# yulong314/multi_camera_calibration

Hardware: AMD Instinct MI355X
Metric: corner residual+Jacobian evals/sec + ms/LM-iter; RMS reproj-err vs ref (higher is better)
Workload: dtype f64; 1 GPU; config4: 4 omnidirectional cameras, 1000 synthetic 11x8-board views (BASELINE.json configs[3]), one Gauss-Newton step per 'step'; model=omnidirectional, cameras=4, views=1000, edges=3958, params=6018, parallelism=photo-sharded x1, transport=none, state_dtype=f32, jacobian_dtype=f64

## Files before the change

### multi_camera_calibration_amd/csrc/mcc_group.hpp

```cpp


template <int MODEL, bool BACK, int L, int GW = 28>
__device__ __forceinline__ void group_prologue(const double* ph, const double* ct, const double* sds, int side,
                                               int sub, double* S, double* P, double* Gb) {
    const double* R1 = ph;
    const double* Jr1 = ph + 9;
    const double* T1 = ph + 18;
    const double* R2 = ct;
    const double* Jl2 = ct + 9;
    const double* T2 = ct + 18;
    double* X = S;
    double* W = S + 15;
    for (int e = sub; e < 12; e += L) {
        if (e < 9) {
            const int i = e / 3, j = e % 3;
            X[e] = dot3_nc(R2[i * 3], R1[j], R2[i * 3 + 1], R1[3 + j], R2[i * 3 + 2], R1[6 + j]);
        } else {
            const int i = e - 9;
            const double q = dot3_nc(R2[i * 3], T1[0], R2[i * 3 + 1], T1[1], R2[i * 3 + 2], T1[2]);
            X[12 + i] = q;
            X[9 + i] = add_nc(q, T2[i]);
        }
    }
    wave_sync_lds();
// ... 351 lines not shown
    const int iter = st->iter;
    const double cn0 = st->cam_normG2, cn1 = st->cam_normX2;
    const int nI = 48 * np, nV = useiv ? m * m + 1 : 0, n = nI + nV;
    if (tid == 0) {
        s_status = useiv ? 0.0 : -1.0;
        s_fail = 0;
    }
    __syncthreads();
    unsigned have = 0;
    auto due = [&](int t) { return t >= nI || t < 48 * a.n_items || t % 48 < 3; };
    const long long t0 = (long long)__builtin_amdgcn_s_memrealtime();
    for (;;) {
        double v[U];
#pragma unroll
        for (int u = 0; u < U; ++u) {
            int t = u * nt + tid;
            t = t < n ? t : n - 1;
            v[u] = ld_sc1(t < nI ? a.item_out + t : la.fiv + (t - nI));
        }
        const double stt = useiv ? ld_sc1(la.fiv + m * m) : -1.0;
        int pend = 0;
#pragma unroll
        for (int u = 0; u < U; ++u) {
            const int t = u * nt + tid;
            if (t >= n || ((have >> u) & 1) || !due(t)) continue;
            if (!fold_valid(v[u])) {
                if (t < nI || t == nI + m * m || !fold_valid(stt) || stt > 0.0) ++pend;
                continue;
            }
            have |= 1u << u;
            if (t < nI) itm[t] = v[u];
            else if (t < nI + m * m) Iv[t - nI] = v[u];
            else s_status = v[u];
        }
        if (!__syncthreads_or(pend)) break;
        if (tid == 0 && (long long)__builtin_amdgcn_s_memrealtime() - t0 >= la.spare_wait) {
            atomicOr(&st->error, kErrWarmTimeout);
            st->done = 1;
            s_fail = 1;
        }
        __syncthreads();
        if (s_fail) return;
    }
#pragma unroll
    for (int u = 0; u < U; ++u) {
        const int t = u * nt + tid;
        if (t < n && ((have >> u) & 1)) fold_empty(t < nI ? a.item_out + t : la.fiv + (t - nI));
    }
    if (tid <= a.nblk) sbi[tid] = bi;
    int err_now = 0;
    for (int k = a.n_items; k < np; ++k) err_now |= itm[48 * k + 2] != 0.0 ? kErrPhotoNotPD : 0;
    __syncthreads();
    SSTAMP(srow, 8, 0);
    schur_finish(a, np, iter, cn0, cn1, err_now, useiv && s_status == (double)(iter + 1), srow, pre);
}
constexpr int kFoldKI = 8;
__device__ __forceinline__ void fold_final_reset(const LinArgs& la, const double* const* src, unsigned have, bool useiv) {
#pragma unroll
    for (int q = 0; q < kFoldKI; ++q)
        if ((have >> q) & 1) fold_empty(const_cast<double*>(src[q]));
    if (threadIdx.x == 0 && useiv) fold_empty(la.fiv + la.fsa.m * la.fsa.m);
}
__device__ __forceinline__ void fold_final_direct(const LinArgs& la, const SolvePre* pre) {
    const SchurArgs& a = la.fsa;
    State* st = a.state;
    const int tid = threadIdx.x, nt = blockDim.x;
    const int m = a.m, nb = m / 6, ntri = m * (m + 1) / 2, np = la.fold_parts, nc = np - a.n_items;
    extern __shared__ __attribute__((aligned(16))) double sm[];
    double* S = sm;
    double* r = sm + m * m;
    double* Iv = sm + m * m + m;
    __shared__ double norms[2];
    __shared__ int s_fail;
    const bool useiv = a.ssinv != nullptr && a.fuse_solve;
    const bool lds = a.fuse_solve && a.peer.nranks == 0;
    long long* srow = a.stamps ? a.stamps + kSchurStampStride * (size_t)np : nullptr;
    SSTAMP(srow, 10, 0);
    const int nent = a.nblk * 48, ivt0 = nent + 2, nivt = nt - ivt0;
    const double* src[kFoldKI];
    int cnt = 0, kind = 0;
    int blk = 0, e = 0;
    if (tid < nent) {
        blk = tid / 48;
        e = tid % 48;
        const int k0 = a.block_items[blk], nk = a.block_items[blk + 1] - k0;
        int b1 = 0;
#pragma unroll
        for (int b = 1; b < 5; ++b)
            if (b < nb && b * nb - b * (b - 1) / 2 <= blk) b1 = b;
        const int b2 = b1 + (blk - (b1 * nb - b1 * (b1 - 1) / 2));
        kind = 1;
        cnt = e >= 36 && b1 != b2 ? 0 : nk;
#pragma unroll
        for (int q = 0; q < kFoldKI; ++q) src[q] = a.item_out + 48 * (size_t)(k0 + (q < nk ? q : 0)) + e;
    } else if (tid < ivt0) {
        const int w = tid - nent;
        kind = 2;
        cnt = 2 * nc;
#pragma unroll
        for (int q = 0; q < kFoldKI; ++q) {
            const int c = q < nc ? q : (q - nc < nc ? q - nc : 0);
            src[q] = a.item_out + 48 * (size_t)(a.n_items + c) + (q < nc ? w : 2);
        }
    } else {
        kind = 3;
        const int j0 = tid - ivt0;
        cnt = 0;
#pragma unroll
        for (int q = 0; q < kFoldKI; ++q) {
            const int j = j0 + q * nivt;
            if (useiv && j < m * m) cnt = q + 1;
            src[q] = la.fiv + (useiv && j < m * m ? j : 0);
        }
    }
    const int iter = st->iter;
    const double cn = kind == 2 && a.rank == 0 ? (tid - nent ? st->cam_normX2 : st->cam_normG2) : 0.0;
    if (tid == 0) s_fail = 0;
    __syncthreads();
    double kv[kFoldKI];
    unsigned have = 0;
    double stt = -1.0;
    const long long t0 = (long long)__builtin_amdgcn_s_memrealtime();
    for (;;) {
        double v[kFoldKI];
#pragma unroll
        for (int q = 0; q < kFoldKI; ++q) v[q] = ld_sc1(((have >> q) & 1) ? la.fiv + m * m : src[q]);
        if (useiv) stt = ld_sc1(la.fiv + m * m);
        int pend = tid == 0 && useiv && !fold_valid(stt) ? 1 : 0;
#pragma unroll
        for (int q = 0; q < kFoldKI; ++q) {
            if (q >= cnt || ((have >> q) & 1)) continue;
            if (fold_valid(v[q])) {
                kv[q] = v[q];
                have |= 1u << q;
            } else if (kind != 3 || !fold_valid(stt) || stt > 0.0) {
                ++pend;
            }
        }
        if (!pend) break;
        if ((long long)__builtin_amdgcn_s_memrealtime() - t0 >= la.spare_wait) {
            s_fail = 1;
            break;
        }
    }
    __shared__ double s_stt;
    if (tid == 0) s_stt = stt;
    __syncthreads();
    if (s_fail) {
        if (tid == 0) {
            atomicOr(&st->error, kErrWarmTimeout);
            st->done = 1;
        }
        return;
    }
    SSTAMP(srow, 8, 0);
    const bool ivok = useiv && s_stt == (double)(iter + 1);
    if (kind == 1 && cnt > 0) {
        double v = 0.0;
#pragma unroll
        for (int q = 0; q < kFoldKI; ++q)
            if (q < cnt) v += kv[q];
        int b1 = 0;
#pragma unroll
        for (int b = 1; b < 5; ++b)
            if (b < nb && b * nb - b * (b - 1) / 2 <= blk) b1 = b;
        const int b2 = b1 + (blk - (b1 * nb - b1 * (b1 - 1) / 2));
        if (e < 36) {
            const int ii = e / 6, jj = e % 6, i = 6 * b1 + ii, j = 6 * b2 + jj;
            if (b1 != b2 || ii <= jj) {
                a.packed[packed_index(i, j, m)] = v;
                if (lds) {
                    S[i * m + j] = v;
                    S[j * m + i] = v;
                }
            }
        } else {
            const int w = (e - 36) / 6, i = 6 * b1 + (e - 36) % 6;
            a.packed[ntri + w * m + i] = v;
            if (lds && w == 0) r[i] = v;
        }
    } else if (kind == 2) {
        const int w = tid - nent;
        double nrm = 0.0, bad = 0.0;
#pragma unroll
        for (int q = 0; q < kFoldKI; ++q) {
            if (q < nc) nrm += kv[q];
            else if (q < 2 * nc) bad += kv[q];
        }
        if (a.rank == 0) nrm += cn;
        if (iter <= 0) nrm = 0.0;
        nrm = photo_flag_norm(bad != 0.0 ? kErrPhotoNotPD : 0, w, nrm);
        norms[w] = nrm;
        a.packed[ntri + 2 * m + w] = nrm;
    } else if (kind == 3 && ivok) {
        const int j0 = tid - ivt0;
#pragma unroll
        for (int q = 0; q < kFoldKI; ++q)
            if (q < cnt) Iv[j0 + q * nivt] = kv[q];
    }
    SSTAMP(srow, 9, 0);
    if (!a.fuse_solve) {
        fold_final_reset(la, src, have, useiv);
        return;
    }
    __syncthreads();
    if (a.peer.nranks > 0) {
        if (!peer_exchange(a.peer, st, a.packed)) {
            fold_final_reset(la, src, have, useiv);
            return;
        }
        for (int t = tid; t < ntri + m; t += nt) {
            const double v = a.packed[t];
            if (t < ntri) {
                int i, j;
                packed_ij(t, m, i, j);
                S[i * m + j] = v;
                S[j * m + i] = v;
            } else {
                r[t - ntri] = v;
            }
        }
        if (tid < 2) norms[tid] = a.packed[ntri + 2 * m + tid];
        __syncthreads();
    }
    SSTAMP(srow, 3, 0);
    SolveCtx sc = a.solve;
    sc.stamps = srow;
    solve_global<false>(sc, S, r, norms[0], norms[1], nullptr, ivok ? Iv : nullptr, pre);
    SSTAMP(srow, 7, 0);
    fold_final_reset(la, src, have, useiv);
    SSTAMP_DRAINED(srow, 15, 0);
}
#ifndef MCC_FOLD_EARLY
#define MCC_FOLD_EARLY 1
#endif
template <int NT>
__device__ __forceinline__ void fold_final(const LinArgs& la) {
    __shared__ SolvePre s_pre;
    const SolvePre* pre = MCC_FOLD_EARLY ? &s_pre : nullptr;
    if (MCC_FOLD_EARLY && la.fsa.fuse_solve) {
        SolveCtx sc = la.fsa.solve;
        sc.stamps = la.fsa.stamps ? la.fsa.stamps + kSchurStampStride * (size_t)la.fold_parts : nullptr;
        solve_prefetch(sc, &s_pre);
    }
    if (NT == 512 && la.fold_direct) {
        fold_final_direct(la, pre);
        return;
    }
    constexpr int UM = kSchurOneLevelLoads * 256 / NT;
    const int n = 48 * la.fold_parts + (la.fsa.ssinv != nullptr ? la.fsa.m * la.fsa.m + 1 : 0);
    if (n <= UM / 2 * NT) fold_final_u<UM / 2>(la, pre);
    else fold_final_u<UM>(la, pre);
}

#ifndef MCC_GROUP_PAIR_THREADS
#define MCC_GROUP_PAIR_THREADS 256
#endif
#ifndef MCC_GROUP_OCC
#define MCC_GROUP_OCC 2
#endif
#ifndef MCC_EDGE_PRIO
#define MCC_EDGE_PRIO 2
#endif
template <int L, int AT>
__device__ __forceinline__ void edge_prio_up() {
    if (L == 32 && MCC_EDGE_PRIO == AT && __builtin_amdgcn_readfirstlane(threadIdx.x) >= 256) __builtin_amdgcn_s_setprio(1);
}
template <int L>
__device__ __forceinline__ void edge_prio_down() {
    if (L == 32 && MCC_EDGE_PRIO != 0) __builtin_amdgcn_s_setprio(0);
}
template <class T>
__device__ __forceinline__ T* pin_global(T* p) {
    __attribute__((address_space(1))) T* g = (__attribute__((address_space(1))) T*)p;
    asm volatile("" : "+s"(g));
    return (T*)g;
}
__device__ __forceinline__ int first_lane(int v) { return __builtin_amdgcn_readfirstlane(v); }
__device__ __forceinline__ double first_lane(double v) {
    return __hiloint2double(first_lane(__double2hiint(v)), first_lane(__double2loint(v)));
}
template <class T>
__device__ __forceinline__ const T& kernarg_at(const int off) {
    typedef const __attribute__((address_space(4))) char* kbytes;
    const __attribute__((address_space(4))) T* p =
        (const __attribute__((address_space(4))) T*)((kbytes)__builtin_amdgcn_kernarg_segment_ptr() + off);
    asm volatile("" : "+s"(p));
    return *(const T*)p;
}
template <int MODEL, bool RATIONAL, int PRISM, bool BACK, int L>
__device__ __forceinline__ bool group_body(State* st, const int* __restrict__ ghdr, const bool fold, const int grp,
                                           const long long t_entry) {
    constexpr int NT = kGroupRound * L, EPW = 64 / L;
    const int tid = threadIdx.x, lane = tid & 63, wave = tid >> 6;
    const int wv = __builtin_amdgcn_readfirstlane(wave);
    const int* __restrict__ hdr = ghdr + (size_t)kGHdrInts * grp;
    int done = first_lane(st->done), pending = first_lane(st->pending);
    double alpha_prev = first_lane(st->alpha);
    int p0 = first_lane(hdr[kGHdrRange]), np = first_lane(hdr[kGHdrRange + 1]);
    int ge0 = first_lane(hdr[kGHdrRange + 2]), gne = first_lane(hdr[kGHdrRange + 3]);
    int q0 = first_lane(hdr[kGHdrRange + 4]), nq = first_lane(hdr[kGHdrRange + 5]);
    int c0 = first_lane(hdr[kGHdrRange + 6]), nc = first_lane(hdr[kGHdrRange + 7]);
    GroupHot hp = kernarg_at<GroupHot>(kGArgHot);
    asm volatile("" ::"s"(done), "s"(pending), "s"(alpha_prev), "s"(p0), "s"(np), "s"(ge0), "s"(gne), "s"(q0), "s"(nq),
                 "s"(c0), "s"(nc), "s"(hp.gpairs), "s"(hp.gcon), "s"(hp.dg), "s"(hp.kintr), "s"(hp.x), "s"(hp.cam_rt),
                 "s"(hp.ds_rt), "s"(hp.zp), "s"(hp.photo_norm), "s"(hp.gblock), "s"(hp.Y), "s"(hp.obj_x), "s"(hp.obj_y),
                 "s"(hp.obj_z), "s"(hp.img_u), "s"(hp.img_v), "s"(hp.stamps), "s"(hp.global_dim), "s"(hp.n_cams));
    asm volatile("" ::"s"(hp.edge_info), "s"(hp.edge_lphoto), "s"(hp.gp_tot), "s"(hp.resid));
    asm volatile("" : "+s"(done), "+s"(pending), "+s"(alpha_prev), "+s"(p0), "+s"(np), "+s"(ge0), "+s"(gne), "+s"(q0),
                 "+s"(nq), "+s"(c0), "+s"(nc), "+s"(hp.global_dim), "+s"(hp.n_cams));
    hp.gpairs = pin_global(hp.gpairs); hp.gcon = pin_global(hp.gcon); hp.dg = pin_global(hp.dg);
    hp.kintr = pin_global(hp.kintr); hp.x = pin_global(hp.x); hp.cam_rt = pin_global(hp.cam_rt);
    hp.ds_rt = pin_global(hp.ds_rt); hp.zp = pin_global(hp.zp); hp.photo_norm = pin_global(hp.photo_norm);
    hp.gblock = pin_global(hp.gblock); hp.Y = pin_global(hp.Y); hp.obj_x = pin_global(hp.obj_x);
    hp.obj_y = pin_global(hp.obj_y); hp.obj_z = pin_global(hp.obj_z); hp.img_u = pin_global(hp.img_u);
    hp.img_v = pin_global(hp.img_v); hp.stamps = pin_global(hp.stamps);
    hp.edge_info = pin_global(hp.edge_info); hp.edge_lphoto = pin_global(hp.edge_lphoto);
    hp.gp_tot = pin_global(hp.gp_tot); hp.resid = pin_global(hp.resid);
    if (done) return false;
    long long* stp = hp.stamps ? hp.stamps + kStampStride * (size_t)grp : nullptr;
    SSTAMP(stp, 0, 0);
#ifdef MCC_DIAG
    if (stp && (tid == 0 || tid == NT - 64)) stp[tid == 0 ? 12 : 13] = t_entry;
#endif
    const int C = hp.n_cams, m = hp.global_dim;
    extern __shared__ __attribute__((aligned(16))) double smem[];
    const GroupLayout GL = group_layout(gne, C, nq, nc);
#ifdef MCC_DIAG
    long long wt0 = 0, wt1 = 0, wt2 = 0, wt3 = 0;
#endif
    double* rec = smem + GL.rec;
    double* s27 = smem + GL.s27;
    double* sLi = smem + GL.sLi;
    double* sv = smem + GL.sv;
    double* sph = smem + GL.sph;
    double* sxn = smem + GL.sxn;
    double* spart = smem + GL.spart;
    double* sdg = smem + GL.sdg;
    double* ctab = smem + GL.ctab;
    double* ktab = smem + GL.ktab;
    double* sds = smem + GL.sds;
    double* sP = smem + GL.sP;
    double* sGb = smem + GL.sGb;
    int* ibase = reinterpret_cast<int*>(smem + GL.ndoubles);
    int4* sInfo = reinterpret_cast<int4*>(ibase + GL.iInfo);
    int* sgb = ibase + GL.iGb;
    int* seq = ibase + GL.iEq;
    int* sph0 = ibase + GL.iPh;
    int4* spq = reinterpret_cast<int4*>(ibase + GL.iPq);
    unsigned* scn = reinterpret_cast<unsigned*>(ibase + GL.iCn);
    float(*sC)[kGChunk][EPW] = reinterpret_cast<float(*)[kGChunk][EPW]>(smem + GL.sU + wave * (5 * kGChunk * EPW / 2));
    GroupChain* sCH = reinterpret_cast<GroupChain*>(smem + GL.sU + wave * (5 * kGChunk * EPW / 2));
    static_assert(EPW * sizeof(GroupChain) <= 5 * kGChunk * EPW * sizeof(float), "k_group chain union");

    const int g = lane % EPW, sub = lane / EPW;
    constexpr int PER = kGChunk / L;
    auto stage_load = [&](float (&v)[PER][5], int sb, int eoff, int cc0, int cn) {
#pragma unroll
        for (int u = 0; u < PER; ++u) {
            const int i = sb + L * u;
            const unsigned c = (unsigned)(eoff + cc0 + (i < cn ? i : 0));
            v[u][0] = hp.obj_x[c];
            v[u][1] = hp.obj_y[c];
            v[u][2] = hp.obj_z[c];
            v[u][3] = hp.img_u[c];
            v[u][4] = hp.img_v[c];
        }
    };
    auto stage_store = [&](const float (&v)[PER][5], int sb, int cn) {
#pragma unroll
        for (int u = 0; u < PER; ++u) {
            const int i = sb + L * u;
            if (i < cn) {
#pragma unroll
                for (int f = 0; f < 5; ++f) sC[f][i][g] = v[u][f];
            }
        }
    };
    auto stage = [&](int eoff, int cc0, int cn) {
        float v[PER][5];
        int sb = sub;
        asm volatile("" : "+v"(sb));
        stage_load(v, sb, eoff, cc0, cn);
        stage_store(v, sb, cn);
    };

    constexpr int CAM0 = NT / 2, DST = CAM0 + 63;
    double om2[3] = {0.0, 0.0, 0.0}, T2[3] = {0.0, 0.0, 0.0};
    const int le0 = wave * EPW + g;
    const int4 info0 = *reinterpret_cast<const int4*>(hdr + kGHdrInfo + 4 * le0);
    int4 rInfo = make_int4(0, 0, 0, 0);
    int rGb = 0, rEq = 0, rPh = 0;
    if (wv == 0) {
        const int t = lane < kGroupRound ? lane : 0;
        rInfo = *reinterpret_cast<const int4*>(hdr + kGHdrInfo + 4 * t);
        rGb = hdr[kGHdrGb + t];
        rEq = hdr[kGHdrEq + t];
        rPh = hdr[kGHdrPhoto + (lane <= kPhotoGroup ? lane : 0)];
    }
    int4 rPq = make_int4(0, 0, 0, 0);
    unsigned rCn = 0;
    double rDg = 0.0, rKt = 0.0;
    if (wv * 64 < nq) rPq = hp.gpairs[q0 + (tid < nq ? tid : 0)];
    if (wv * 64 < nc) rCn = hp.gcon[c0 + (tid < nc ? tid : 0)];
    if (wv * 64 < m) rDg = hp.dg[tid < m ? tid : 0];
    if (wv * 64 < kGIntr * C) rKt = hp.kintr[tid < kGIntr * C ? tid : 0];
    float rCam[6] = {0.f, 0.f, 0.f, 0.f, 0.f, 0.f};
    double rDs[6] = {0.0, 0.0, 0.0, 0.0, 0.0, 0.0};
    if (wv == CAM0 / 64) {
        const int c = lane < C ? lane : 0;
        const float* src = MODEL == MCC_MODEL_DOUBLESIDE ? hp.cam_rt + 6 * c : hp.x + 6 * (c > 0 ? c - 1 : 0);
        if (BACK && MODEL == MCC_MODEL_DOUBLESIDE) src = tid == DST ? hp.x : src;
#pragma unroll
        for (int k = 0; k < 6; ++k) rCam[k] = src[k];
        if (BACK && MODEL != MCC_MODEL_DOUBLESIDE) {
#pragma unroll
            for (int k = 0; k < 6; ++k) rDs[k] = hp.ds_rt[k];
        }
    }
    float xo = 0.f;
    double zk = 0.0;
    const int pq = (tid - 192) / 6, pk = (tid - 192) % 6;
    const bool ptask = tid >= 192 && pq < np;
    double2 pn0 = make_double2(0.0, 0.0);
    if (wv == 3) {
        const size_t pi = ptask ? 6 * (size_t)(p0 + pq) + pk : 0;
        xo = hp.x[m + pi];
        if (pending) zk = hp.zp[pi];
        else if (fold) pn0 = *reinterpret_cast<const double2*>(hp.photo_norm + (ptask && pk == 0 ? 2 * (size_t)(p0 + pq) : 0));
    }
    double y0[6] = {0.0, 0.0, 0.0, 0.0, 0.0, 0.0};
    int gb0 = -1;
    if (pending && wv * 64 < 6 * gne) {
        const bool act = tid < 6 * gne;
        const int le = act ? tid / 6 : 0, k = act ? tid % 6 : 0;
        gb0 = hp.gblock[ge0 + le];
        const double* Ye = hp.Y + 36 * (size_t)(ge0 + le);
#pragma unroll
        for (int i = 0; i < 6; ++i) y0[i] = Ye[6 * i + k];
    }
    float cv0[PER][5];
    int sb0 = sub;
    asm volatile("" : "+v"(sb0));
    const int cn0 = min(info0.w, kGChunk);
    __builtin_amdgcn_sched_barrier(0);
    stage_load(cv0, sb0, info0.z, 0, cn0);
    __builtin_amdgcn_sched_barrier(0);
#pragma unroll
    for (int k = 0; k < 6; ++k) asm volatile("" : "+v"(rCam[k]));
    if (wv == 0) {
        if (lane < kGroupRound && lane < gne) {
            sInfo[lane] = rInfo;
            sgb[lane] = rGb;
            seq[lane] = rEq;
        }
        if (lane <= np) sph0[lane] = rPh;
    }
    if (tid < nq) spq[tid] = rPq;
    if (tid < nc) scn[tid] = rCn;
    if (tid < m) sdg[tid] = rDg;
    if (tid < kGIntr * C) ktab[tid] = rKt;
    if (tid >= CAM0 && tid < CAM0 + C) {
        const bool fixed0 = MODEL != MCC_MODEL_DOUBLESIDE && tid == CAM0;
#pragma unroll
        for (int k = 0; k < 3; ++k) {
            om2[k] = fixed0 ? 0.0 : (double)rCam[k];
            T2[k] = fixed0 ? 0.0 : (double)rCam[3 + k];
        }
    } else if (BACK && tid == DST) {
#pragma unroll
        for (int k = 0; k < 3; ++k) {
            om2[k] = MODEL == MCC_MODEL_DOUBLESIDE ? (double)rCam[k] : rDs[k];
            T2[k] = MODEL == MCC_MODEL_DOUBLESIDE ? (double)rCam[3 + k] : rDs[3 + k];
        }
    }
#pragma unroll 1
    for (int t = kGroupRound + tid; t < gne; t += NT) {
        sInfo[t] = hp.edge_info[ge0 + t];
        sgb[t] = hp.gblock[ge0 + t];
        seq[t] = hp.edge_lphoto[ge0 + t];
    }
#pragma unroll 1
    for (int t = NT + tid; t < nq; t += NT) spq[t] = hp.gpairs[q0 + t];
#pragma unroll 1
    for (int t = NT + tid; t < nc; t += NT) scn[t] = hp.gcon[c0 + t];
#pragma unroll 1
    for (int t = NT + tid; t < kGIntr * C; t += NT) ktab[t] = hp.kintr[t];
    __syncthreads();
    SSTAMP(stp, 1, 0);
    const LinArgs& a = kernarg_at<LinArgs>(kGArgLin);
    if (pending) {
        for (int t = tid; t < 6 * gne; t += NT) {
            const int le = t / 6, k = t % 6;
            int gbl = gb0;
            double y[6];
            if (t == tid) {
#pragma unroll
                for (int i = 0; i < 6; ++i) y[i] = y0[i];
            } else {
                gbl = sgb[le];
                const double* Ye = hp.Y + 36 * (size_t)(ge0 + le);
#pragma unroll
                for (int i = 0; i < 6; ++i) y[i] = Ye[6 * i + k];
            }
            const double* d = sdg + 6 * (gbl < 0 ? 0 : gbl);
            double sk = 0.0;
#pragma unroll
            for (int i = 0; i < 6; ++i) sk += y[i] * d[i];
            spart[6 * le + k] = gbl < 0 ? 0.0 : sk;
        }
    }
    __syncthreads();
    if (tid >= CAM0 && tid < CAM0 + C) {
        const int c = tid - CAM0;
        Rot r2;
        rodrigues_v2m(om2, r2);
        double J[9];
        so3_jac(om2, r2, +1.0, J);
        double* ct = ctab + 24 * c;
#pragma unroll
        for (int k = 0; k < 9; ++k) { ct[k] = r2.R[k]; ct[9 + k] = J[k]; }
#pragma unroll
        for (int k = 0; k < 3; ++k) ct[18 + k] = T2[k];
    } else if (BACK && tid == DST) {
        Rot rd;
        rodrigues_v2m(om2, rd);
        double J[9];
        so3_jac(om2, rd, -1.0, J);
#pragma unroll
        for (int k = 0; k < 9; ++k) { sds[k] = rd.R[k]; sds[9 + k] = J[k]; }
#pragma unroll
        for (int k = 0; k < 3; ++k) sds[18 + k] = T2[k];
    }
    if (ptask) {
        float xn = xo;
        double Gk = 0.0;
        if (pending) {
            double t = zk;
            for (int le = sph0[pq]; le < sph0[pq + 1]; ++le) t -= spart[6 * le + pk];
            const float G = (float)(alpha_prev * t);
            xn = xo + G;
            hp.x[m + 6 * (size_t)(p0 + pq) + pk] = xn;
            Gk = (double)G;
        }
        sxn[16 * pq + pk] = (double)xn;
        sxn[16 * pq + 8 + pk] = Gk;
    }
    wave_sync_lds();
    if (ptask && pk == 0) {
        const double* xs = sxn + 16 * pq;
        if (pending) {
            double g2 = 0.0, x2 = 0.0;
#pragma unroll
            for (int q = 0; q < 6; ++q) {
                g2 += xs[8 + q] * xs[8 + q];
                x2 += xs[q] * xs[q];
            }
            hp.photo_norm[2 * (size_t)(p0 + pq)] = g2;
            hp.photo_norm[2 * (size_t)(p0 + pq) + 1] = x2;
            pn0 = make_double2(g2, x2);
        }
        if (fold) {
            sxn[16 * pq + 6] = pn0.x;
            sxn[16 * pq + 7] = pn0.y;
        }
        const double om1[3] = {xs[0], xs[1], xs[2]};
        Rot r1;
        rodrigues_v2m(om1, r1);
        double* ph = sph + 24 * pq;
        so3_jac(om1, r1, -1.0, ph + 9);
#pragma unroll
        for (int k = 0; k < 9; ++k) ph[k] = r1.R[k];
#pragma unroll
        for (int k = 0; k < 3; ++k) ph[18 + k] = xs[3 + k];
    }
    __syncthreads();
    SSTAMP(stp, 2, 0);
    WSTAMP(wt0);
    stage_store(cv0, sb0, cn0);

    for (int rb = 0; rb < gne; rb += kGroupRound) {
        const int es = wave * EPW + g, le = rb + es;
        const bool ev = le < gne;
        const int4 info = ev ? sInfo[le] : make_int4(0, 0, 0, 0);
        const int cam = info.x;
        double* P = sP + kGRecP * es;
        double* Gbe = sGb + 56 * es;
        edge_prio_up<L, 1>();
        if (rb > 0 && ev) stage(info.z, 0, min(info.w, kGChunk));
        if (ev) {
            group_prologue<MODEL, BACK, L>(sph + 24 * seq[le], ctab + 24 * cam, sds, info.y, sub, rec + kGRec * le, P, Gbe);
            const double* kt = ktab + kGIntr * cam;
            for (int k = sub; k < (PRISM == 2 ? 27 : 18); k += L) P[12 + k] = kt[k];
        }
        wave_sync_lds();
        if (rb == 0) SSTAMP(stp, 3, 0);
        if (rb == 0) WSTAMP(wt1);
        edge_prio_up<L, 2>();
        double acc[32];
#pragma unroll
        for (int q = 0; q < 32; ++q) acc[q] = 0.0;
        const int nn = info.w;
        for (int cc0 = 0;; cc0 += kGChunk) {
            if (cc0 >= nn) break;
            const int cn = min(nn - cc0, kGChunk);
            if (cc0 > 0) {
                wave_sync_lds();
                stage(info.z, cc0, cn);
                wave_sync_lds();
            }
#pragma unroll 1
            for (int i = sub; i < cn; i += L) {
                int po = 0;
                asm volatile("" : "+v"(po));
                const double* Pq = P + po;
                double R[9], T[3], kd[12];
#pragma unroll
                for (int q = 0; q < 9; ++q) R[q] = Pq[q];
#pragma unroll
                for (int q = 0; q < 3; ++q) T[q] = Pq[9 + q];
#pragma unroll
                for (int q = 0; q < 12; ++q) kd[q] = Pq[18 + q];
                const double fx = Pq[12], fy = Pq[13], cx = Pq[14], cy = Pq[15], sk = Pq[16], xi = Pq[17];
                const double X = sC[0][i][g], Y = sC[1][i][g], Z = sC[2][i][g];
                const float ou = sC[3][i][g], ov = sC[4][i][g];
                double Yr[3], D[6];
                float u, v;
                if (MODEL == MCC_MODEL_OMNI)
                    omni_corner(R, T, kd, fx, fy, cx, cy, sk, xi, X, Y, Z, Yr, u, v, D);
                else
                    pinhole_corner<RATIONAL, PRISM>(R, T, kd, fx, fy, cx, cy, X, Y, Z, Yr, u, v, D, Pq + 30);
                const float euf = ou - u, evf = ov - v;
                if (hp.resid) {
                    const size_t c = (size_t)info.z + cc0 + i;
                    hp.resid[2 * c] = euf;
                    hp.resid[2 * c + 1] = evf;
                }
                const double eu = euf, ev2 = evf;
                double ju[6], jv[6];
                ju[0] = Yr[1] * D[2] - Yr[2] * D[1];
                ju[1] = Yr[2] * D[0] - Yr[0] * D[2];
                ju[2] = Yr[0] * D[1] - Yr[1] * D[0];
                ju[3] = D[0]; ju[4] = D[1]; ju[5] = D[2];
                jv[0] = Yr[1] * D[5] - Yr[2] * D[4];
                jv[1] = Yr[2] * D[3] - Yr[0] * D[5];
                jv[2] = Yr[0] * D[4] - Yr[1] * D[3];
                jv[3] = D[3]; jv[4] = D[4]; jv[5] = D[5];
                int q = 0;
#pragma unroll
                for (int r = 0; r < 6; ++r)
#pragma unroll
                    for (int s2 = r; s2 < 6; ++s2, ++q) acc[q] = fma(jv[r], jv[s2], fma(ju[r], ju[s2], acc[q]));
#pragma unroll
                for (int r = 0; r < 6; ++r) acc[21 + r] = fma(jv[r], ev2, fma(ju[r], eu, acc[21 + r]));
            }
        }
        if (rb == 0) SSTAMP(stp, 4, 0);
        if (rb == 0) WSTAMP(wt2);
        edge_prio_up<L, 3>();
        int tq = lane;
        asm volatile("" : "+v"(tq));
        strided_reduce_scatter<L>(acc, tq);
        const int gq = tq % EPW, sq = tq / EPW;
        const int base = strided_rs_base<L>(tq);
        wave_sync_lds();
        {
            GroupChain& CW = sCH[gq];
#pragma unroll
            for (int q = 0; q < 32 / L; ++q) {
                const int idx = base + q;
                if (idx < 21) {
                    int r, s2;
                    tri6(idx, r, s2);
                    CW.A[r * 6 + s2] = acc[q];
                    CW.A[s2 * 6 + r] = acc[q];
                } else if (idx < 27) {
                    CW.B[idx - 21] = acc[q];
                }
            }
        }
        wave_sync_lds();
        {
            const int eq = rb + wave * EPW + gq;
            group_chain(sCH[gq], sGb + 56 * (wave * EPW + gq), sq, eq < gne, rec + kGRec * (eq < gne ? eq : 0));
        }
        wave_sync_lds();
        edge_prio_down<L>();
        if (rb == 0) SSTAMP(stp, 5, 0);
        if (rb == 0) WSTAMP(wt3);
    }
#ifdef MCC_DIAG
    if (stp && lane == 0 && wave < 16) {
        __builtin_amdgcn_sched_barrier(0);
        stp[16 + wave] = (long long)MCC_DIAG_CLOCK();
        __builtin_amdgcn_sched_barrier(0);
    }
    if (stp && lane == 0 && wave < 8) {
        const long long m21 = (1ll << 21) - 1;
        stp[24 + wave] = ((wt1 - wt0) & m21) | (((wt2 - wt0) & m21) << 21) | (((wt3 - wt0) & m21) << 42);
    }
#endif
    __syncthreads();
    SSTAMP(stp, 6, 0);

    constexpr int ES = kGRec;
    double* sE = rec;
    if (tid < 27 * np) {
        const int q = tid / 27, col27 = tid % 27;
        double s = 0.0;
        for (int le = sph0[q]; le < sph0[q + 1]; ++le) s += rec[kGRec * le + 64 + col27];
        s27[28 * q + col27] = s;
    }
    __syncthreads();
    SSTAMP(stp, 7, 0);
    if (tid < np) {
        const int q = tid, photo = p0 + q;
        double A[21], gs[6], Lm[6][6], Li[6][6];
        const double2* S2 = reinterpret_cast<const double2*>(s27 + 28 * q);
#pragma unroll
        for (int k = 0; k < 14; ++k) {
            const double2 w = S2[k];
            if (2 * k < 21) A[2 * k] = w.x; else gs[2 * k - 21] = w.x;
            if (2 * k + 1 < 21) A[2 * k + 1] = w.y; else if (2 * k + 1 < 27) gs[2 * k + 1 - 21] = w.y;
        }
        bool bad = false;
        double idg[6];
#pragma unroll
        for (int j = 0; j < 6; ++j) {
            double d = A[6 * j - j * (j - 1) / 2];
#pragma unroll
            for (int k = 0; k < j; ++k) d -= Lm[j][k] * Lm[j][k];
            bad |= !(d > 0.0);
            const double sd = sqrt(d > 0.0 ? d : 1.0);
            const double is = 1.0 / sd;
            Lm[j][j] = sd;
            idg[j] = is;
#pragma unroll
            for (int i = j + 1; i < 6; ++i) {
                double t = A[6 * j - j * (j - 1) / 2 + (i - j)];
#pragma unroll
                for (int k = 0; k < j; ++k) t -= Lm[i][k] * Lm[j][k];
                Lm[i][j] = t * is;
            }
        }
#pragma unroll
        for (int j = 0; j < 6; ++j) {
#pragma unroll
            for (int i = 0; i < 6; ++i) {
                if (i < j) { Li[i][j] = 0.0; continue; }
                double t = i == j ? 1.0 : 0.0;
#pragma unroll
                for (int k = j; k < i; ++k) t -= Lm[i][k] * Li[k][j];
                Li[i][j] = t * idg[i];
            }
        }
        double vv[6];
#pragma unroll
        for (int i = 0; i < 6; ++i) {
            double t = 0.0;
#pragma unroll
            for (int k = 0; k <= i; ++k) t += Li[i][k] * gs[k];
            vv[i] = t;
        }
#pragma unroll
        for (int j = 0; j < 6; ++j) {
            double t = 0.0;
#pragma unroll
            for (int i = j; i < 6; ++i) t += Li[i][j] * vv[i];
            hp.zp[6 * (size_t)photo + j] = t;
            hp.gp_tot[6 * (size_t)photo + j] = gs[j];
            sv[6 * q + j] = vv[j];
        }
        double2* L2 = reinterpret_cast<double2*>(sLi + 36 * q);
#pragma unroll
        for (int k = 0; k < 18; ++k) L2[k] = make_double2(Li[(2 * k) / 6][(2 * k) % 6], Li[(2 * k + 1) / 6][(2 * k + 1) % 6]);
        if (bad || photo == a.fault_photo) atomicOr(&st->error, kErrPhotoNotPD);
        if (fold) {
            double* fw = a.fnorm + 4 * (size_t)photo;
            st_sc1_x2(fw, sxn[16 * q + 6], sxn[16 * q + 7]);
            st_sc1(fw + 2, bad || photo == a.fault_photo ? 1.0 : 0.0);
        }
    }
    __syncthreads();
    SSTAMP(stp, 8, 0);
    for (int t = tid; t < 6 * gne; t += NT) {
        const int le = t / 6, i = t % 6;
        double h[6], li[36], u[6], y[6];
        double2* H2 = reinterpret_cast<double2*>(sE + ES * le + 22 + 6 * i);
        const double2* I2 = reinterpret_cast<const double2*>(sLi + 36 * seq[le]);
#pragma unroll
        for (int q = 0; q < 3; ++q) { const double2 w = H2[q]; h[2 * q] = w.x; h[2 * q + 1] = w.y; }
#pragma unroll
        for (int q = 0; q < 18; ++q) { const double2 w = I2[q]; li[2 * q] = w.x; li[2 * q + 1] = w.y; }
        const bool gl = sgb[le] >= 0;
#pragma unroll
        for (int j = 0; j < 6; ++j) {
            double w = 0.0;
#pragma unroll
            for (int k = 0; k <= j; ++k) w += h[k] * li[6 * j + k];
            u[j] = gl ? w : 0.0;
        }
#pragma unroll
        for (int j = 0; j < 6; ++j) {
            double w = 0.0;
#pragma unroll
            for (int k = j; k < 6; ++k) w += u[k] * li[6 * k + j];
            y[j] = w;
        }
        double2* G2 = reinterpret_cast<double2*>(hp.Y + 36 * (size_t)(ge0 + le) + 6 * i);
#pragma unroll
        for (int q = 0; q < 3; ++q) {
            H2[q] = make_double2(u[2 * q], u[2 * q + 1]);
            G2[q] = make_double2(y[2 * q], y[2 * q + 1]);
        }
    }
    __syncthreads();
    SSTAMP(stp, 9, 0);
    int H = 1;
    while (H < 32 && 6 * nq * 2 * H <= (NT < MCC_GROUP_PAIR_THREADS ? NT : MCC_GROUP_PAIR_THREADS)) H *= 2;
    for (int t = tid; t < 6 * nq * H; t += NT) {
        const int h = t % H, k = t / H / 6, i0 = (t / H) % 6;
        const int4 pqv = spq[k];
        const bool diag = (pqv.z & 2) != 0;
        double acc[6], racc = 0.0, jacc = 0.0;
#pragma unroll
        for (int j = 0; j < 6; ++j) acc[j] = 0.0;
#pragma unroll 1
        for (int c = pqv.x + h; c < pqv.x + pqv.y; c += H) {
            const unsigned w = scn[c];
            const int ea = w & 255, eb = (w >> 8) & 255, q = w >> 17;
            const bool self = (w >> 16) & 1;
            const double2* Y2 = reinterpret_cast<const double2*>(sE + ES * ea + 22 + 6 * i0);
            const double2* B2 = reinterpret_cast<const double2*>(sE + ES * eb + 22);
            double y[6];
#pragma unroll
            for (int qq = 0; qq < 3; ++qq) { const double2 v = Y2[qq]; y[2 * qq] = v.x; y[2 * qq + 1] = v.y; }
            const double* Hgg = sE + ES * ea;
#pragma unroll
            for (int j = 0; j < 6; ++j) {
                double hb[6];
#pragma unroll
                for (int qq = 0; qq < 3; ++qq) { const double2 v = B2[3 * j + qq]; hb[2 * qq] = v.x; hb[2 * qq + 1] = v.y; }
                double d = 0.0;
#pragma unroll
                for (int kk = 0; kk < 6; ++kk) d += y[kk] * hb[kk];
                double hv = 0.0;
                if (self) {
                    const int rr = i0 < j ? i0 : j, cc = i0 < j ? j : i0;
                    hv = Hgg[rr * 6 - rr * (rr - 1) / 2 + (cc - rr)];
                }
                acc[j] += self ? hv - d : -d;
            }
            if (diag && self) {
                double d = 0.0;
#pragma unroll
                for (int kk = 0; kk < 6; ++kk) d += y[kk] * sv[6 * q + kk];
                const double gg = sE[ES * ea + 58 + i0];
                racc += gg - d;
                jacc += gg;
            }
        }
        for (int o = 1; o < H; o <<= 1) {
#pragma unroll
            for (int j = 0; j < 6; ++j) acc[j] += __shfl_xor(acc[j], o);
            racc += __shfl_xor(racc, o);
            jacc += __shfl_xor(jacc, o);
        }
        if (h == 0) {
            double* out = a.pairprod + (size_t)pqv.w;
#ifdef MCC_SLOT_PLAIN
#pragma unroll
            for (int j = 0; j < 6; ++j) out[i0 * 6 + j] = acc[j];
            if (diag) {
                out[36 + i0] = racc;
                out[42 + i0] = jacc;
            }
#else
#pragma unroll
            for (int j = 0; j < 6; j += 2) st_sc1_x2(out + i0 * 6 + j, acc[j], acc[j + 1]);
            if (diag) {
                st_sc1(out + 36 + i0, racc);
                st_sc1(out + 42 + i0, jacc);
            }
#endif
        }
    }
#ifdef MCC_DIAG
    asm volatile("s_waitcnt vmcnt(0)" ::: "memory");
    __syncthreads();
    SSTAMP(stp, 10, 0);
#endif
    return true;
}

template <int MODEL, bool RATIONAL, int PRISM, bool BACK, int L, bool FIRST = false>
__global__ __launch_bounds__(kGroupRound * L, MCC_GROUP_OCC * 16 / L) void k_group(
    State* st, const int* ghdr, const int n_pgroups, const unsigned flags, const int n_items, const int fold_parts,
    long long, long long, long long, long long, LinArgs, GroupHot) {
    constexpr int NT = kGroupRound * L;
    static_assert(L == 16 || L == 32, "k_group: 16 or 32 lanes per edge");
    static_assert(GSame<decltype(&k_group<MODEL, RATIONAL, PRISM, BACK, L, FIRST>), GroupKernelFn>::v,
                  "k_group's parameters are GroupKernelFn's: kernarg_at's offsets are computed from that list");
    long long t_entry = 0;
    WSTAMP(t_entry);
    const int tid = threadIdx.x;
    const bool spare = (flags & kGLeadSsinv) != 0, fold = (flags & kGLeadFold) != 0;
    int grp = blockIdx.x;
    if (FIRST) {
        const int nlead = (int)gridDim.x - n_pgroups;
        grp = grp < nlead ? n_pgroups + grp : grp - nlead;
    }
    if (spare && grp == n_pgroups) {
        extern __shared__ __attribute__((aligned(16))) double smem_spare[];
        small_inverse(kernarg_at<LinArgs>(kGArgLin), smem_spare, false);
        return;
    }
    int task;
    if (fold && grp > n_pgroups - (spare ? 0 : 1)) {
        if (st->done) return;
        task = grp - n_pgroups - (spare ? 1 : 0);
    } else {
        if (!group_body<MODEL, RATIONAL, PRISM, BACK, L>(st, ghdr, fold, grp, t_entry) || PRISM == 2 ||
            !(flags & kGLeadFoldDyn))
            return;
        __shared__ int s_task;
        __syncthreads();
        if (tid == 0) {
            int* ticket = kernarg_at<LinArgs>(kGArgLin).fold_ticket;
            const int t = __hip_atomic_fetch_add(ticket, 1, __ATOMIC_RELAXED, __HIP_MEMORY_SCOPE_AGENT);
            if (t == n_pgroups - 1) __hip_atomic_store(ticket, 0, __ATOMIC_RELAXED, __HIP_MEMORY_SCOPE_AGENT);
            s_task = t;
        }
        __syncthreads();
        task = s_task;
    }
    const LinArgs& a = kernarg_at<LinArgs>(kGArgLin);
    if (task < n_items) fold_item(a, task);
    else if (task < fold_parts) fold_chunk(a, task - n_items);
    else if (task == fold_parts) fold_final<NT>(a);
}

#ifndef MCC_PREP4_WAVES
#define MCC_PREP4_WAVES 2
#endif
template <int MODEL, bool BACK>
__global__ __launch_bounds__(64, MCC_PREP4_WAVES) void k_prep4(LinArgs a) {
    const State* st = a.state;
    const int tid = threadIdx.x, grp = blockIdx.x;
    const int done = st->done, pending = st->pending;
    const double alpha_prev = st->alpha;
    const int p0 = a.prep_ptr[grp], np = a.prep_ptr[grp + 1] - p0;
    const int ge0 = a.prep_edge[grp], gne = a.prep_edge[grp + 1] - ge0;
    if (done) return;
    long long* stp = a.stamps ? a.stamps + kStampStride * (size_t)grp + 8 : nullptr;
    SSTAMP(stp, 0, 0);
    const int C = a.n_cams, m = a.global_dim;
    extern __shared__ __attribute__((aligned(16))) double smem[];
    const PrepLayout PL = prep_layout(C, BACK);
    double* tab = smem + PL.tab;
    double* S = smem + PL.S;
    double* spart = S;
    double* sdg = smem + PL.sdg;
    double* sxn = smem + PL.sxn;
    double* scam = smem + PL.scam;
    int* ib = reinterpret_cast<int*>(smem + PL.ndoubles);
    int4* sInfo = reinterpret_cast<int4*>(ib + PL.iInfo);
    int* sgb = ib + PL.iGb;
    int* sph0 = ib + PL.iPh;
    constexpr int SW = BACK ? 84 : 42;
    for (int t = tid; t < m; t += 64) sdg[t] = a.dg[t];
    for (int t = tid; t < 6 * C; t += 64) {
        const int c = t / 6, k = t % 6;
        scam[t] = MODEL == MCC_MODEL_DOUBLESIDE ? (double)a.cam_rt[t]
                                                : (c == 0 ? 0.0 : (double)a.x[6 * (c - 1) + k]);
    }
    if (BACK && tid < 6) scam[6 * C + tid] = MODEL == MCC_MODEL_DOUBLESIDE ? (double)a.x[tid] : a.ds_rt[tid];
    if (tid <= np) sph0[tid] = a.photo_ptr[p0 + tid] - ge0;
    for (int t = tid; t < gne; t += 64) {
        sInfo[t] = a.edge_info[ge0 + t];
        sgb[t] = a.gblock[ge0 + t];
    }
    const int pq = tid / 6, pk = tid % 6;
    const bool ptask = pq < np;
    float xo = 0.f;
    double zk = 0.0;
    double2 pn0 = make_double2(0.0, 0.0);
    if (ptask) {
        xo = a.x[m + 6 * (size_t)(p0 + pq) + pk];
        if (pending) zk = a.zp[6 * (size_t)(p0 + pq) + pk];
        else if (a.fold && pk == 0) pn0 = *reinterpret_cast<const double2*>(a.photo_norm + 2 * (size_t)(p0 + pq));
    }
    double y0[6];
    int gb0 = -1;
    if (pending && tid < 6 * gne) {
        const int le = tid / 6, k = tid % 6;
        gb0 = a.gblock[ge0 + le];
        const double* Ye = a.Y + 36 * (size_t)(ge0 + le);
#pragma unroll
        for (int i = 0; i < 6; ++i) y0[i] = Ye[6 * i + k];
    }
    wave_sync_lds();
    if (pending) {
        for (int t = tid; t < 6 * gne; t += 64) {
            const int le = t / 6, k = t % 6;
            int gbl = gb0;
            double y[6];
            if (t == tid) {
#pragma unroll
                for (int i = 0; i < 6; ++i) y[i] = y0[i];
            } else {
                gbl = sgb[le];
                const double* Ye = a.Y + 36 * (size_t)(ge0 + le);
#pragma unroll
                for (int i = 0; i < 6; ++i) y[i] = Ye[6 * i + k];
            }
            const double* d = sdg + 6 * (gbl < 0 ? 0 : gbl);
            double sk = 0.0;
#pragma unroll
            for (int i = 0; i < 6; ++i) sk += y[i] * d[i];
            spart[6 * le + k] = gbl < 0 ? 0.0 : sk;
        }
    }
    wave_sync_lds();
    if (ptask) {
        float xn = xo;
        double Gk = 0.0;
        if (pending) {
            double t = zk;
            for (int le = sph0[pq]; le < sph0[pq + 1]; ++le) t -= spart[6 * le + pk];
            const float G = (float)(alpha_prev * t);
            xn = xo + G;
            a.x[m + 6 * (size_t)(p0 + pq) + pk] = xn;
            Gk = (double)G;
        }
        sxn[16 * pq + pk] = (double)xn;
        sxn[16 * pq + 8 + pk] = Gk;
    }
    wave_sync_lds();
    SSTAMP(stp, 1, 0);
    if (pending && ptask && pk == 0) {
        const double* xs = sxn + 16 * pq;
        double g2 = 0.0, x2 = 0.0;
#pragma unroll
        for (int q = 0; q < 6; ++q) {
            g2 += xs[8 + q] * xs[8 + q];
            x2 += xs[q] * xs[q];
        }
        a.photo_norm[2 * (size_t)(p0 + pq)] = g2;
        a.photo_norm[2 * (size_t)(p0 + pq) + 1] = x2;
    }
    for (int t = tid; t < np + C + (BACK ? 1 : 0); t += 64) {
        const double* src;
        double* out;
        double sgn;
        if (t < np) {
            src = sxn + 16 * t; out = tab + 24 * t; sgn = -1.0;
        } else if (t < np + C) {
            src = scam + 6 * (t - np); out = tab + 24 * (kPrepPhotos + t - np); sgn = 1.0;
        } else {
            src = scam + 6 * C; out = tab + 24 * (kPrepPhotos + C); sgn = -1.0;
        }
        const double om[3] = {src[0], src[1], src[2]};
        Rot r;
        rodrigues_v2m(om, r);
        double J[9];
        so3_jac(om, r, sgn, J);
#pragma unroll
        for (int k = 0; k < 9; ++k) { out[k] = r.R[k]; out[9 + k] = J[k]; }
#pragma unroll
        for (int k = 0; k < 3; ++k) out[18 + k] = src[3 + k];
    }
    wave_sync_lds();
    SSTAMP(stp, 2, 0);
    const int es = tid >> 2, sub = tid & 3;
    for (int rb = 0; rb < gne; rb += kPrepEdges) {
        const int le = rb + es;
        if (le < gne) {
            const int4 info = sInfo[le];
            int q = 0;
            while (q + 1 < np && sph0[q + 1] <= le) ++q;
            const size_t e = (size_t)ge0 + le;
            group_prologue<MODEL, BACK, 4, 27>(tab + 24 * q, tab + 24 * (kPrepPhotos + info.x), tab + 24 * (kPrepPhotos + C),
                                               info.y, sub, S + SW * es, a.erec + 12 * e, a.echain + 54 * e);
        }
        wave_sync_lds();
    }
#ifdef MCC_DIAG
    asm volatile("s_waitcnt vmcnt(0)" ::: "memory");
#endif
    SSTAMP(stp, 3, 0);
}
```

Baseline: 14.51 billion corner evals/s.

## Defer global stores past pair products and prefetch LDS indices across barriers

Moves the per-photo zp/gp_tot/fnorm/error writes and the first-round Y stores to the end of the group body, so global store latency overlaps the pair-product phase instead of sitting before barriers. Hoists the LDS reads for the first task (seq, sgb, spq, scn) ahead of the preceding __syncthreads, and software-prefetches the next connection word inside the pair loop. The pair-loop index math now uses shifts instead of modulo. The cost is extra live registers (zq, gs, yl, prefetched values), which may raise register pressure and lower occupancy.

```diff
diff --git a/multi_camera_calibration_amd/csrc/mcc_group.hpp b/multi_camera_calibration_amd/csrc/mcc_group.hpp
--- a/multi_camera_calibration_amd/csrc/mcc_group.hpp
+++ b/multi_camera_calibration_amd/csrc/mcc_group.hpp
@@ -677,13 +677,19 @@
     int q0 = first_lane(hdr[kGHdrRange + 4]), nq = first_lane(hdr[kGHdrRange + 5]);
     int c0 = first_lane(hdr[kGHdrRange + 6]), nc = first_lane(hdr[kGHdrRange + 7]);
     GroupHot hp = kernarg_at<GroupHot>(kGArgHot);
+    const LinArgs& a = kernarg_at<LinArgs>(kGArgLin);
+    double* fnorm = a.fnorm;
+    double* pairprod = a.pairprod;
+    int fault_photo = a.fault_photo;
     asm volatile("" ::"s"(done), "s"(pending), "s"(alpha_prev), "s"(p0), "s"(np), "s"(ge0), "s"(gne), "s"(q0), "s"(nq),
                  "s"(c0), "s"(nc), "s"(hp.gpairs), "s"(hp.gcon), "s"(hp.dg), "s"(hp.kintr), "s"(hp.x), "s"(hp.cam_rt),
                  "s"(hp.ds_rt), "s"(hp.zp), "s"(hp.photo_norm), "s"(hp.gblock), "s"(hp.Y), "s"(hp.obj_x), "s"(hp.obj_y),
                  "s"(hp.obj_z), "s"(hp.img_u), "s"(hp.img_v), "s"(hp.stamps), "s"(hp.global_dim), "s"(hp.n_cams));
-    asm volatile("" ::"s"(hp.edge_info), "s"(hp.edge_lphoto), "s"(hp.gp_tot), "s"(hp.resid));
+    asm volatile("" ::"s"(hp.edge_info), "s"(hp.edge_lphoto), "s"(hp.gp_tot), "s"(hp.resid), "s"(fnorm), "s"(pairprod),
+                 "s"(fault_photo));
     asm volatile("" : "+s"(done), "+s"(pending), "+s"(alpha_prev), "+s"(p0), "+s"(np), "+s"(ge0), "+s"(gne), "+s"(q0),
-                 "+s"(nq), "+s"(c0), "+s"(nc), "+s"(hp.global_dim), "+s"(hp.n_cams));
+                 "+s"(nq), "+s"(c0), "+s"(nc), "+s"(hp.global_dim), "+s"(hp.n_cams), "+s"(fault_photo));
+    fnorm = pin_global(fnorm); pairprod = pin_global(pairprod);
     hp.gpairs = pin_global(hp.gpairs); hp.gcon = pin_global(hp.gcon); hp.dg = pin_global(hp.dg);
     hp.kintr = pin_global(hp.kintr); hp.x = pin_global(hp.x); hp.cam_rt = pin_global(hp.cam_rt);
     hp.ds_rt = pin_global(hp.ds_rt); hp.zp = pin_global(hp.zp); hp.photo_norm = pin_global(hp.photo_norm);
@@ -863,7 +869,6 @@
     for (int t = NT + tid; t < kGIntr * C; t += NT) ktab[t] = hp.kintr[t];
     __syncthreads();
     SSTAMP(stp, 1, 0);
-    const LinArgs& a = kernarg_at<LinArgs>(kGArgLin);
     if (pending) {
         for (int t = tid; t < 6 * gne; t += NT) {
             const int le = t / 6, k = t % 6;
@@ -1080,6 +1085,13 @@
 
     constexpr int ES = kGRec;
     double* sE = rec;
+    int hs = 0;
+    while (hs < 5 && 6 * nq * (2 << hs) <= (NT < MCC_GROUP_PAIR_THREADS ? NT : MCC_GROUP_PAIR_THREADS)) ++hs;
+    const int H = 1 << hs;
+    const bool ut0 = tid < 6 * gne, pt0 = tid < 6 * nq * H;
+    const int ule0 = ut0 ? tid / 6 : 0;
+    const int ueq0 = seq[ule0], ugb0 = sgb[ule0];
+    const int4 pqv0 = spq[pt0 ? (tid >> hs) / 6 : 0];
     if (tid < 27 * np) {
         const int q = tid / 27, col27 = tid % 27;
         double s = 0.0;
@@ -1088,10 +1100,16 @@
     }
     __syncthreads();
     SSTAMP(stp, 7, 0);
+    const unsigned pw0 = scn[pt0 && (tid & (H - 1)) < pqv0.y ? pqv0.x + (tid & (H - 1)) : 0];
+    double zq[6] = {0.0, 0.0, 0.0, 0.0, 0.0, 0.0}, gs[6] = {0.0, 0.0, 0.0, 0.0, 0.0, 0.0};
+    double ng2 = 0.0, nx2 = 0.0;
+    bool npd = false;
     if (tid < np) {
         const int q = tid, photo = p0 + q;
-        double A[21], gs[6], Lm[6][6], Li[6][6];
+        double A[21], Lm[6][6], Li[6][6];
         const double2* S2 = reinterpret_cast<const double2*>(s27 + 28 * q);
+        ng2 = sxn[16 * q + 6];
+        nx2 = sxn[16 * q + 7];
 #pragma unroll
         for (int k = 0; k < 14; ++k) {
             const double2 w = S2[k];
@@ -1142,32 +1160,26 @@
             double t = 0.0;
 #pragma unroll
             for (int i = j; i < 6; ++i) t += Li[i][j] * vv[i];
-            hp.zp[6 * (size_t)photo + j] = t;
-            hp.gp_tot[6 * (size_t)photo + j] = gs[j];
+            zq[j] = t;
             sv[6 * q + j] = vv[j];
         }
         double2* L2 = reinterpret_cast<double2*>(sLi + 36 * q);
 #pragma unroll
         for (int k = 0; k < 18; ++k) L2[k] = make_double2(Li[(2 * k) / 6][(2 * k) % 6], Li[(2 * k + 1) / 6][(2 * k + 1) % 6]);
-        if (bad || photo == a.fault_photo) atomicOr(&st->error, kErrPhotoNotPD);
-        if (fold) {
-            double* fw = a.fnorm + 4 * (size_t)photo;
-            st_sc1_x2(fw, sxn[16 * q + 6], sxn[16 * q + 7]);
-            st_sc1(fw + 2, bad || photo == a.fault_photo ? 1.0 : 0.0);
-        }
+        npd = bad || photo == fault_photo;
     }
     __syncthreads();
     SSTAMP(stp, 8, 0);
-    for (int t = tid; t < 6 * gne; t += NT) {
+    auto uy_task = [&](const int t, const int eq, const int gb, double (&y)[6]) {
         const int le = t / 6, i = t % 6;
-        double h[6], li[36], u[6], y[6];
+        double h[6], li[36], u[6];
         double2* H2 = reinterpret_cast<double2*>(sE + ES * le + 22 + 6 * i);
-        const double2* I2 = reinterpret_cast<const double2*>(sLi + 36 * seq[le]);
+        const double2* I2 = reinterpret_cast<const double2*>(sLi + 36 * eq);
 #pragma unroll
         for (int q = 0; q < 3; ++q) { const double2 w = H2[q]; h[2 * q] = w.x; h[2 * q + 1] = w.y; }
 #pragma unroll
         for (int q = 0; q < 18; ++q) { const double2 w = I2[q]; li[2 * q] = w.x; li[2 * q + 1] = w.y; }
-        const bool gl = sgb[le] >= 0;
+        const bool gl = gb >= 0;
 #pragma unroll
         for (int j = 0; j < 6; ++j) {
             double w = 0.0;
@@ -1182,27 +1194,35 @@
             for (int k = j; k < 6; ++k) w += u[k] * li[6 * k + j];
             y[j] = w;
         }
-        double2* G2 = reinterpret_cast<double2*>(hp.Y + 36 * (size_t)(ge0 + le) + 6 * i);
-#pragma unroll
-        for (int q = 0; q < 3; ++q) {
-            H2[q] = make_double2(u[2 * q], u[2 * q + 1]);
-            G2[q] = make_double2(y[2 * q], y[2 * q + 1]);
-        }
+#pragma unroll
+        for (int q = 0; q < 3; ++q) H2[q] = make_double2(u[2 * q], u[2 * q + 1]);
+    };
+    auto store_y = [&](const int t, const double (&y)[6]) {
+        double2* G2 = reinterpret_cast<double2*>(hp.Y + 6 * (size_t)(6 * ge0 + t));
+#pragma unroll
+        for (int q = 0; q < 3; ++q) G2[q] = make_double2(y[2 * q], y[2 * q + 1]);
+    };
+    double yl[6] = {0.0, 0.0, 0.0, 0.0, 0.0, 0.0};
+    if (ut0) {
+        uy_task(tid, ueq0, ugb0, yl);
+    }
+#pragma unroll 1
+    for (int t = tid + NT; t < 6 * gne; t += NT) {
+        double y[6];
+        uy_task(t, seq[t / 6], sgb[t / 6], y);
+        store_y(t, y);
     }
     __syncthreads();
     SSTAMP(stp, 9, 0);
-    int H = 1;
-    while (H < 32 && 6 * nq * 2 * H <= (NT < MCC_GROUP_PAIR_THREADS ? NT : MCC_GROUP_PAIR_THREADS)) H *= 2;
-    for (int t = tid; t < 6 * nq * H; t += NT) {
-        const int h = t % H, k = t / H / 6, i0 = (t / H) % 6;
-        const int4 pqv = spq[k];
+    auto pair_task = [&](const int t, const int4 pqv, unsigned w) {
+        const int h = t & (H - 1), i0 = (t >> hs) % 6;
         const bool diag = (pqv.z & 2) != 0;
         double acc[6], racc = 0.0, jacc = 0.0;
 #pragma unroll
         for (int j = 0; j < 6; ++j) acc[j] = 0.0;
 #pragma unroll 1
         for (int c = pqv.x + h; c < pqv.x + pqv.y; c += H) {
-            const unsigned w = scn[c];
+            const unsigned wn = c + H < pqv.x + pqv.y ? scn[c + H] : 0u;
             const int ea = w & 255, eb = (w >> 8) & 255, q = w >> 17;
             const bool self = (w >> 16) & 1;
             const double2* Y2 = reinterpret_cast<const double2*>(sE + ES * ea + 22 + 6 * i0);
@@ -1234,6 +1254,7 @@
                 racc += gg - d;
                 jacc += gg;
             }
+            w = wn;
         }
         for (int o = 1; o < H; o <<= 1) {
 #pragma unroll
@@ -1242,7 +1263,7 @@
             jacc += __shfl_xor(jacc, o);
         }
         if (h == 0) {
-            double* out = a.pairprod + (size_t)pqv.w;
+            double* out = pairprod + (size_t)pqv.w;
 #ifdef MCC_SLOT_PLAIN
 #pragma unroll
             for (int j = 0; j < 6; ++j) out[i0 * 6 + j] = acc[j];
@@ -1258,6 +1279,29 @@
                 st_sc1(out + 42 + i0, jacc);
             }
 #endif
+        }
+    };
+    if (pt0) pair_task(tid, pqv0, pw0);
+#pragma unroll 1
+    for (int t = tid + NT; t < 6 * nq * H; t += NT) {
+        const int4 pqv = spq[(t >> hs) / 6];
+        pair_task(t, pqv, scn[(t & (H - 1)) < pqv.y ? pqv.x + (t & (H - 1)) : 0]);
+    }
+    SSTAMP(stp, 11, 0);
+    if (tid < np) {
+        if (fold) {
+            double* fw = fnorm + 4 * (size_t)(p0 + tid);
+            st_sc1_x2(fw, ng2, nx2);
+            st_sc1(fw + 2, npd ? 1.0 : 0.0);
+        }
+        if (npd) atomicOr(&st->error, kErrPhotoNotPD);
+    }
+    if (ut0) store_y(tid, yl);
+    if (tid < np) {
+#pragma unroll
+        for (int j = 0; j < 6; ++j) {
+            hp.zp[6 * (size_t)(p0 + tid) + j] = zq[j];
+            hp.gp_tot[6 * (size_t)(p0 + tid) + j] = gs[j];
         }
     }
 #ifdef MCC_DIAG
```

Result: faster. 14.80 billion corner evals/s, median of 6 (+1.9%).
